# san-soucie/gdrf

Hardware: AMD Instinct MI355X
Metric: ELBO steps/sec (+ achieved HBM GB/s on K_nm) at N=1e6,M=512,K=10,V=50 (higher is better)
Workload: dtype f32; 1 GPU; configs[3] at 1 GPU(s): N=1000000 synthetic 2-D lattice (1000x1000), V=50, K=10, M=512 (32x16 grid inducing points), rbf kernel, Adam lr=1e-3, Trace_ELBO, 1 particle, jitter=1e-06, observations sharded over ranks; N=1000000, M=512, K=10, V=50, D=2, rows_per_rank=1000000, jitter_level=2, stores_T=False, mfma_mode=f16x3

## Files before the change

### gdrf_amd/csrc/gemm_tn_topics1.h

```cpp
#pragma once
#include <utility>
#include "gemm_tn_topics.h"

namespace gdrf {

template <int... Is, class F> __device__ __forceinline__ void static_for_impl(std::integer_sequence<int, Is...>, F&& f) {
  (f(std::integral_constant<int, Is>{}), ...);
}
template <int N, class F> __device__ __forceinline__ void static_for(F&& f) { static_for_impl(std::make_integer_sequence<int, N>{}, f); }

constexpr int TN1_CH = 64;
constexpr int TN1_XBLK = 1056;
constexpr int TN1_X_BYTES = 16 * TN1_XBLK;
constexpr int TN1_VROWS = 12;
constexpr int TN1_V_BYTES = TN1_VROWS * TN1_CH * 4;
constexpr int TN1_NBUF = 3;

__device__ __forceinline__ void glds4_asm(const void* gsrc, unsigned lds_dst) {
  asm volatile("s_mov_b32 m0, %1\n\ts_nop 0\n\tglobal_load_lds_dword %0, off" : : "v"(gsrc), "s"(lds_dst) : "memory");
}

__device__ __forceinline__ void glds4_asm_s(const void* sbase, unsigned voff, unsigned lds_dst) {
  asm volatile("s_mov_b32 m0, %2\n\ts_nop 0\n\tglobal_load_lds_dword %0, %1" : : "v"(voff), "s"(sbase), "s"(lds_dst) : "memory");
}

__global__ void tn1_scale_rows_kernel(const float* __restrict__ vbar, int64_t ldk, int64_t nrows, float* __restrict__ vs, int64_t lds,
                                      const float* __restrict__ sc, int sidx_v) {
  const int k = blockIdx.y;
  const float scale = sc[sidx_v + 2 * k];
  for (int64_t n = (int64_t)blockIdx.x * blockDim.x + threadIdx.x; n < lds; n += (int64_t)gridDim.x * blockDim.x)
    vs[(int64_t)k * lds + n] = n < nrows ? vbar[(int64_t)k * ldk + n] * scale : 0.0f;
}

constexpr int TN2_A_BYTES = 2 * 2 * 32 * 128 * 2;
constexpr int TN2_BUF = TN2_A_BYTES + TN1_X_BYTES + TN1_V_BYTES;
constexpr int TN2_DMA_PER_CHUNK = 15;
constexpr int tn2_lds_bytes() { return TN1_NBUF * TN2_BUF; }

__host__ __device__ inline int tn2_ntiles_half(int ncols) {
  const int nI = (ncols + 127) / 128, nJ = (ncols + 63) / 64;
  int t = 0;
  for (int I = 0; I < nI; ++I) t += (2 * I + 1 < nJ) ? 1 : 0;
  return t;
}
template <int AMIN>
__global__ __launch_bounds__(256, 1) void tn_topics_w2_kernel(TNTopicsArgs g) {
  using E = _Float16;
  using V8 = f16x8;
  using V4 = f16x4;
  constexpr int KT = TNT_KT, PIECE = 32 * 128, KA = 8;
  static_assert(KT == 10, "register plan below is for 10 topics");
  extern __shared__ __attribute__((aligned(16))) char smem[];
  const int tid = threadIdx.x, lane = tid & 63;
  const int w = __builtin_amdgcn_readfirstlane(tid >> 6);
  const int lr = lane & 15, lg = lane >> 4;
  const int kgroups = (g.K + KT - 1) / KT;
  const unsigned units = (unsigned)(g.ntiles * kgroups), bid = blockIdx.x;
  unsigned u; int sp;
  if ((g.nsplit & 7) == 0) { const unsigned idx = bid >> 3; sp = (int)(idx / units) * 8 + (int)(bid & 7u); u = idx % units; }
  else { sp = (int)(bid / units); u = bid % units; }
  const int tile = (int)(u % (unsigned)g.ntiles), gk = (int)(u / (unsigned)g.ntiles);
  int I = 0, J = tile;
  if (AMIN == 4) { I = tile; J = 2 * tile + 1; }
  else {
    const int nJ = (g.ncols + 63) / 64;
    for (;; ++I) { const int cnt = 2 * I + 1 < nJ ? 2 * I + 1 : nJ; if (J < cnt) break; J -= cnt; }
  }
  const int i0 = I * 128, j0 = J * 64;
  const int k0 = gk * KT, kg = min(KT, g.K - k0);
  const int64_t r0 = (int64_t)sp * g.rows_per_split;
  int64_t r1 = r0 + g.rows_per_split; if (r1 > g.nrows) r1 = g.nrows;
  const int nch = r0 < r1 ? (int)((r1 - r0 + TN1_CH - 1) / TN1_CH) : 0;
  const bool col_ok = (j0 + 16 * w) < g.ncols;
  const int bj = 2 * J + (w >> 1);

  f32x4 accA[KA][8], accV[KT - KA][8];
#pragma unroll
  for (int a = 0; a < 8; ++a) {
#pragma unroll
    for (int k = 0; k < KA; ++k) accA[k][a] = f32x4{0, 0, 0, 0};
#pragma unroll
    for (int k = 0; k < KT - KA; ++k) accV[k][a] = f32x4{0, 0, 0, 0};
  }

  const unsigned lds0 = lds_addr(smem);
  auto dma_edge = [&](int c, int buf) {
    const unsigned base = lds0 + (unsigned)(buf * TN2_BUF);
    const int64_t n0 = r0 + (int64_t)c * TN1_CH;
#pragma unroll
    for (int s = 0; s < 2; ++s)
#pragma unroll
      for (int h = 0; h < 2; ++h) {
        const int rb = w + 4 * h, k = 4 * rb + (lane >> 4);
        const int c8 = (lane & 15) ^ (tnb_code(k) << 1);
        int64_t n = n0 + 32 * s + k;
        n = n < g.nrows ? n : g.nrows - 1;
        const int col = (i0 + 8 * c8 < g.ncols) ? i0 + 8 * c8 : 0;
#pragma unroll
        for (int p = 0; p < 2; ++p)
          glds16_asm(g.Ah + p * g.a_stride + n * g.lda + col, base + (unsigned)((s * 2 + p) * PIECE * 2 + rb * 1024));
      }
    const int xcol = (j0 + 4 * (lane & 15) < g.ncols) ? j0 + 4 * (lane & 15) : 0;
#pragma unroll
    for (int t = 0; t < 4; ++t) {
      const int blk = 4 * w + t;
      int64_t n = n0 + 4 * blk + (lane >> 4);
      n = n < g.nrows ? n : g.nrows - 1;
      glds16_asm(g.B + n * g.ldb + xcol, base + (unsigned)(TN2_A_BYTES + blk * TN1_XBLK));
    }
#pragma unroll
    for (int t = 0; t < 3; ++t) {
      const int kk = w + 4 * t, ks = kk < kg ? kk : kg - 1;
      glds4_asm(g.vbar + (int64_t)(k0 + ks) * g.ldk + n0 + lane, base + (unsigned)(TN2_A_BYTES + TN1_X_BYTES + kk * TN1_CH * 4));
    }
  };
  unsigned voff_a, voff_x;
  {
    const int k = 4 * w + (lane >> 4);
    const int c8 = (lane & 15) ^ (tnb_code(k) << 1);
    const int col = (i0 + 8 * c8 < g.ncols) ? i0 + 8 * c8 : 0;
    voff_a = (unsigned)(((int64_t)(lane >> 4) * g.lda + col) * 2);
    const int xcol = (j0 + 4 * (lane & 15) < g.ncols) ? j0 + 4 * (lane & 15) : 0;
    voff_x = (unsigned)(((int64_t)(lane >> 4) * g.ldb + xcol) * 4);
  }
  const unsigned voff_v = (unsigned)lane * 4u;
  auto dma_is_edge = [&](int c) { return r0 + (int64_t)c * TN1_CH + TN1_CH > g.nrows; };
  auto dma_piece = [&](int c, int buf, int q) {
    const int64_t n0 = r0 + (int64_t)c * TN1_CH;
    const unsigned base = lds0 + (unsigned)(buf * TN2_BUF);
    if (q < 8) {
      const int s = q >> 2, h = (q >> 1) & 1, p = q & 1;
      glds16_asm_s(g.Ah + p * g.a_stride + (n0 + 32 * s + 16 * h + 4 * w) * g.lda, voff_a, base + (unsigned)((s * 2 + p) * PIECE * 2 + (w + 4 * h) * 1024));
    } else if (q < 12) {
      const int t = q - 8;
      glds16_asm_s(g.B + (n0 + 4 * (4 * w + t)) * g.ldb, voff_x, base + (unsigned)(TN2_A_BYTES + (4 * w + t) * TN1_XBLK));
    } else {
      const int kk = w + 4 * (q - 12), ks = kk < kg ? kk : kg - 1;
      glds4_asm_s(g.vbar + (int64_t)(k0 + ks) * g.ldk + n0, voff_v, base + (unsigned)(TN2_A_BYTES + TN1_X_BYTES + kk * TN1_CH * 4));
    }
  };
  auto dma = [&](int c, int buf) {
    if (dma_is_edge(c)) { dma_edge(c, buf); return; }
#pragma unroll
    for (int q = 0; q < TN2_DMA_PER_CHUNK; ++q) dma_piece(c, buf, q);
  };
  const int fq = lr >> 2, fp = lr & 3, fcode = ((lg & 1) << 2) | fq;
  const int fbase = (8 * lg + fq) * 32 + fp;
  auto frag = [&](const E* img, int g16) -> V8 {
    const int seg = fbase + ((g16 ^ fcode) << 2);
    const V4 lo = tr_read(img + seg * 4);
    const V4 hi = tr_read(img + (seg + 128) * 4);
    return __builtin_shufflevector(lo, hi, 0, 1, 2, 3, 4, 5, 6, 7);
  };
  const unsigned kmask = 0xffffe000u;
  const float k2048 = 2048.0f;
  auto split_piece = [&](int q, float xa, float xb, float va, float vb, float& y0, float& y1, float& h0, float& h1, unsigned& H, unsigned& L) {
    if (q == 0) asm volatile("v_mul_f32 %0, %2, %3\n\tv_mul_f32 %1, %4, %5" : "=&v"(y0), "=&v"(y1) : "v"(xa), "v"(va), "v"(xb), "v"(vb));
    if (q == 1) asm volatile("v_and_b32 %0, %2, %3\n\tv_and_b32 %1, %2, %4" : "=&v"(h0), "=&v"(h1) : "s"(kmask), "v"(y0), "v"(y1));
    if (q == 2) asm volatile("v_sub_f32 %0, %0, %2\n\tv_sub_f32 %1, %1, %3" : "+v"(y0), "+v"(y1) : "v"(h0), "v"(h1));
    if (q == 3) asm volatile("v_cvt_pkrtz_f16_f32 %0, %2, %3\n\tv_mul_f32 %1, %4, %1" : "=&v"(H), "+v"(y0) : "v"(h0), "v"(h1), "s"(k2048));
    if (q == 4) asm volatile("v_mul_f32 %1, %3, %1\n\tv_cvt_pk_f16_f32 %0, %2, %1" : "=&v"(L), "+v"(y1) : "v"(y0), "s"(k2048));
  };
  auto mfma_a = [&](f32x4& acc, const V8& a, const V8& b) { asm volatile("v_mfma_f32_16x16x32_f16 %0, %1, %2, %0" : "+a"(acc) : "v"(a), "v"(b)); };
  auto mfma_v = [&](f32x4& acc, const V8& a, const V8& b) { asm volatile("v_mfma_f32_16x16x32_f16 %0, %1, %2, %0" : "+v"(acc) : "v"(a), "v"(b)); };
  auto wait_next = [&](bool two_ahead) {
    if (two_ahead) asm volatile("s_waitcnt vmcnt(%0) lgkmcnt(0)" :: "n"(TN2_DMA_PER_CHUNK) : "memory");
    else asm volatile("s_waitcnt vmcnt(0) lgkmcnt(0)" ::: "memory");
  };

  if (nch > 0) {
    constexpr int NA = 8 - AMIN, NM = 3 * NA, NPS = NM - 2;
    dma(0, 0);
    if (nch > 1) dma(1, 1);
    wait_next(nch > 1);
    gdrf_raw_barrier();
    int buf = 0, bn = 2;
    for (int c = 0; c < nch; ++c) {
      const bool two = c + 2 < nch;
      const bool spread = two && !dma_is_edge(c + 2);
      if (two && !spread) dma_edge(c + 2, bn);
      const E* As = reinterpret_cast<const E*>(smem + buf * TN2_BUF);
      const float* xs = reinterpret_cast<const float*>(smem + buf * TN2_BUF + TN2_A_BYTES);
      const float* vt = reinterpret_cast<const float*>(smem + buf * TN2_BUF + TN2_A_BYTES + TN1_X_BYTES);
      V8 fah[8], fal[8], fa2[8];
#pragma unroll
      for (int a = AMIN; a < 8; ++a) { fah[a] = frag(As, a); fal[a] = frag(As + PIECE, a); }
      float xv[2][8];
#pragma unroll
      for (int s = 0; s < 2; ++s)
#pragma unroll
        for (int e = 0; e < 8; ++e) xv[s][e] = xs[(8 * s + 2 * lg + (e >> 2)) * (TN1_XBLK / 4) + (e & 3) * 64 + 16 * w + lr];
      constexpr int NST = 2 * KT;
      f32x4 vv[3][2];
      auto load_vv = [&](int t) {
        const int s = t / KT, k = t % KT;
        vv[t % 3][0] = *reinterpret_cast<const f32x4*>(vt + k * TN1_CH + 32 * s + 8 * lg);
        vv[t % 3][1] = *reinterpret_cast<const f32x4*>(vt + k * TN1_CH + 32 * s + 8 * lg + 4);
      };
      unsigned Hh[2][4], Ll[2][4];
      float y0, y1, h0, h1;
      auto piece = [&](int t, int q20) {
        const int s = t / KT, g2 = q20 / 5;
        const f32x4 v = vv[t % 3][g2 >> 1];
        split_piece(q20 % 5, xv[s][2 * g2], xv[s][2 * g2 + 1], v[2 * (g2 & 1)], v[2 * (g2 & 1) + 1], y0, y1, h0, h1, Hh[t & 1][g2], Ll[t & 1][g2]);
      };
      load_vv(0);
      load_vv(1);
#pragma unroll
      for (int a = AMIN; a < 8; ++a) fa2[a] = fah[a] * (E)0.00048828125f;
#pragma unroll
      for (int q = 0; q < 20; ++q) piece(0, q);
      typedef unsigned u32x4 __attribute__((ext_vector_type(4)));
      V8 fbh = __builtin_bit_cast(V8, u32x4{Hh[0][0], Hh[0][1], Hh[0][2], Hh[0][3]});
      V8 fbl = __builtin_bit_cast(V8, u32x4{Ll[0][0], Ll[0][1], Ll[0][2], Ll[0][3]});
      asm volatile("s_nop 1" : "+v"(fbh), "+v"(fbl));
      static_for<NST>([&](auto tc) {
        constexpr int t = decltype(tc)::value;
        constexpr int s = t / KT, k = t % KT;
        if (k == 0) {
          if (s == 1) {
#pragma unroll
            for (int a = AMIN; a < 8; ++a) { fah[a] = frag(As + 2 * PIECE, a); fal[a] = frag(As + 3 * PIECE, a); }
#pragma unroll
            for (int a = AMIN; a < 8; ++a) fa2[a] = fah[a] * (E)0.00048828125f;
          }
          if (AMIN == 0) asm volatile("s_nop 1" : "+v"(fa2[0]), "+v"(fa2[1]), "+v"(fa2[2]), "+v"(fa2[3]), "+v"(fa2[4]), "+v"(fa2[5]), "+v"(fa2[6]), "+v"(fa2[7]));
          else asm volatile("s_nop 1" : "+v"(fa2[4]), "+v"(fa2[5]), "+v"(fa2[6]), "+v"(fa2[7]));
        }
        if (t + 2 < NST) load_vv(t + 2);
        const V8 fbh_t = fbh, fbl_t = fbl;
        static_for<NM>([&](auto mc) {
          constexpr int m = decltype(mc)::value;
          constexpr int x = m / NA, a = AMIN + m % NA;
          const V8& fa = x == 0 ? fa2[a] : (x == 1 ? fal[a] : fah[a]);
          const V8& fb = x == 0 ? fbl_t : fbh_t;
          if (k < KA) mfma_a(accA[k < KA ? k : 0][a], fa, fb); else mfma_v(accV[k >= KA ? k - KA : 0][a], fa, fb);
          if (m < NPS && t + 1 < NST) {
#pragma unroll
            for (int q = m * 20 / NPS; q < (m + 1) * 20 / NPS; ++q) piece(t + 1, q);
          }
          if (m == NPS - 1 && t + 1 < NST) {
            fbh = __builtin_bit_cast(V8, u32x4{Hh[(t + 1) & 1][0], Hh[(t + 1) & 1][1], Hh[(t + 1) & 1][2], Hh[(t + 1) & 1][3]});
            fbl = __builtin_bit_cast(V8, u32x4{Ll[(t + 1) & 1][0], Ll[(t + 1) & 1][1], Ll[(t + 1) & 1][2], Ll[(t + 1) & 1][3]});
            asm volatile("" : "+v"(fbh), "+v"(fbl));
          }
          if (m == NM - 2 && spread && t < TN2_DMA_PER_CHUNK) dma_piece(c + 2, bn, t);
        });
      });
      wait_next(two);
      gdrf_raw_barrier();
      buf = buf == 2 ? 0 : buf + 1;
      bn = bn == 2 ? 0 : bn + 1;
    }
  }
  asm volatile("s_nop 15\n\ts_nop 15" ::: "memory");
  if (!col_ok) return;
  const float una = g.sc[g.sidx_a + 1];
#pragma unroll
  for (int k = 0; k < KT; ++k) {
    if (k < kg) {
      const float un = una * g.sc[g.sidx_v + 2 * (k0 + k) + 1];
      float* out = g.slab + ((int64_t)sp * g.K + k0 + k) * (int64_t)g.ncols * g.ncols;
#pragma unroll
      for (int a = 0; a < 8; ++a) {
        if (4 * I + (a >> 1) < bj) continue;
#pragma unroll
        for (int r = 0; r < 4; ++r) {
          const int i = i0 + 16 * a + 4 * lg + r;
          const int j = j0 + 16 * w + lr;
          const float v = k < KA ? accA[k < KA ? k : 0][a][r] : accV[k >= KA ? k - KA : 0][a][r];
          if (i < g.ncols && j < g.ncols) out[(int64_t)i * g.ncols + j] = v * un;
        }
      }
    }
  }
}

}
```

Measured before the change: 25.12 steps/s.

## Software-pipeline operand prefetch across chunk boundaries in topics GEMM

Hoists the fragment registers out of the chunk loop and prefetches the next chunk's A fragments, x values and v vectors from LDS during the current chunk's last MFMA steps. The wait and barrier move earlier, to step NST-2. This removes the per-chunk prologue where LDS reads and the split pieces ran with no MFMA overlap. In exchange, more registers stay live and the barrier placement is more delicate, with a risk of races or spills.

```diff
diff --git a/gdrf_amd/csrc/gemm_tn_topics1.h b/gdrf_amd/csrc/gemm_tn_topics1.h
--- a/gdrf_amd/csrc/gemm_tn_topics1.h
+++ b/gdrf_amd/csrc/gemm_tn_topics1.h
@@ -170,11 +170,50 @@
 
   if (nch > 0) {
     constexpr int NA = 8 - AMIN, NM = 3 * NA, NPS = NM - 2;
+    constexpr int NST = 2 * KT;
+    typedef unsigned u32x4 __attribute__((ext_vector_type(4)));
+    V8 fah[8], fal[8], fa2[8];
+    float xv[2][8];
+    f32x4 vv[3][2];
+    unsigned Hh[2][4], Ll[2][4];
+    float y0, y1, h0, h1;
+    V8 fbh, fbl;
+    auto xread = [&](const float* xs, int s, int e) {
+      return xs[(8 * s + 2 * lg + (e >> 2)) * (TN1_XBLK / 4) + (e & 3) * 64 + 16 * w + lr];
+    };
+    auto load_vv = [&](const float* vt, int t) {
+      const int s = t / KT, k = t % KT;
+      vv[t % 3][0] = *reinterpret_cast<const f32x4*>(vt + k * TN1_CH + 32 * s + 8 * lg);
+      vv[t % 3][1] = *reinterpret_cast<const f32x4*>(vt + k * TN1_CH + 32 * s + 8 * lg + 4);
+    };
+    auto piece = [&](int t, int q20) {
+      const int s = t / KT, g2 = q20 / 5;
+      const f32x4 v = vv[t % 3][g2 >> 1];
+      split_piece(q20 % 5, xv[s][2 * g2], xv[s][2 * g2 + 1], v[2 * (g2 & 1)], v[2 * (g2 & 1) + 1], y0, y1, h0, h1, Hh[t & 1][g2], Ll[t & 1][g2]);
+    };
     dma(0, 0);
     if (nch > 1) dma(1, 1);
     wait_next(nch > 1);
     gdrf_raw_barrier();
-    int buf = 0, bn = 2;
+    {
+      const E* As = reinterpret_cast<const E*>(smem);
+      const float* xs = reinterpret_cast<const float*>(smem + TN2_A_BYTES);
+      const float* vt = reinterpret_cast<const float*>(smem + TN2_A_BYTES + TN1_X_BYTES);
+#pragma unroll
+      for (int a = AMIN; a < 8; ++a) { fah[a] = frag(As, a); fal[a] = frag(As + PIECE, a); }
+#pragma unroll
+      for (int e = 0; e < 8; ++e) xv[0][e] = xread(xs, 0, e);
+      load_vv(vt, 0);
+      load_vv(vt, 1);
+#pragma unroll
+      for (int a = AMIN; a < 8; ++a) fa2[a] = fah[a] * (E)0.00048828125f;
+#pragma unroll
+      for (int q = 0; q < 20; ++q) piece(0, q);
+      fbh = __builtin_bit_cast(V8, u32x4{Hh[0][0], Hh[0][1], Hh[0][2], Hh[0][3]});
+      fbl = __builtin_bit_cast(V8, u32x4{Ll[0][0], Ll[0][1], Ll[0][2], Ll[0][3]});
+      asm volatile("s_nop 1" : "+v"(fbh), "+v"(fbl));
+    }
+    int buf = 0, b1 = 1, bn = 2;
     for (int c = 0; c < nch; ++c) {
       const bool two = c + 2 < nch;
       const bool spread = two && !dma_is_edge(c + 2);
@@ -182,75 +221,54 @@
       const E* As = reinterpret_cast<const E*>(smem + buf * TN2_BUF);
       const float* xs = reinterpret_cast<const float*>(smem + buf * TN2_BUF + TN2_A_BYTES);
       const float* vt = reinterpret_cast<const float*>(smem + buf * TN2_BUF + TN2_A_BYTES + TN1_X_BYTES);
-      V8 fah[8], fal[8], fa2[8];
-#pragma unroll
-      for (int a = AMIN; a < 8; ++a) { fah[a] = frag(As, a); fal[a] = frag(As + PIECE, a); }
-      float xv[2][8];
-#pragma unroll
-      for (int s = 0; s < 2; ++s)
-#pragma unroll
-        for (int e = 0; e < 8; ++e) xv[s][e] = xs[(8 * s + 2 * lg + (e >> 2)) * (TN1_XBLK / 4) + (e & 3) * 64 + 16 * w + lr];
-      constexpr int NST = 2 * KT;
-      f32x4 vv[3][2];
-      auto load_vv = [&](int t) {
-        const int s = t / KT, k = t % KT;
-        vv[t % 3][0] = *reinterpret_cast<const f32x4*>(vt + k * TN1_CH + 32 * s + 8 * lg);
-        vv[t % 3][1] = *reinterpret_cast<const f32x4*>(vt + k * TN1_CH + 32 * s + 8 * lg + 4);
-      };
-      unsigned Hh[2][4], Ll[2][4];
-      float y0, y1, h0, h1;
-      auto piece = [&](int t, int q20) {
-        const int s = t / KT, g2 = q20 / 5;
-        const f32x4 v = vv[t % 3][g2 >> 1];
-        split_piece(q20 % 5, xv[s][2 * g2], xv[s][2 * g2 + 1], v[2 * (g2 & 1)], v[2 * (g2 & 1) + 1], y0, y1, h0, h1, Hh[t & 1][g2], Ll[t & 1][g2]);
-      };
-      load_vv(0);
-      load_vv(1);
-#pragma unroll
-      for (int a = AMIN; a < 8; ++a) fa2[a] = fah[a] * (E)0.00048828125f;
-#pragma unroll
-      for (int q = 0; q < 20; ++q) piece(0, q);
-      typedef unsigned u32x4 __attribute__((ext_vector_type(4)));
-      V8 fbh = __builtin_bit_cast(V8, u32x4{Hh[0][0], Hh[0][1], Hh[0][2], Hh[0][3]});
-      V8 fbl = __builtin_bit_cast(V8, u32x4{Ll[0][0], Ll[0][1], Ll[0][2], Ll[0][3]});
-      asm volatile("s_nop 1" : "+v"(fbh), "+v"(fbl));
+      const E* As_n = reinterpret_cast<const E*>(smem + b1 * TN2_BUF);
+      const float* xs_n = reinterpret_cast<const float*>(smem + b1 * TN2_BUF + TN2_A_BYTES);
+      const float* vt_n = reinterpret_cast<const float*>(smem + b1 * TN2_BUF + TN2_A_BYTES + TN1_X_BYTES);
       static_for<NST>([&](auto tc) {
         constexpr int t = decltype(tc)::value;
         constexpr int s = t / KT, k = t % KT;
+        constexpr int tn = (t + 1) % NST;
         if (k == 0) {
-          if (s == 1) {
-#pragma unroll
-            for (int a = AMIN; a < 8; ++a) { fah[a] = frag(As + 2 * PIECE, a); fal[a] = frag(As + 3 * PIECE, a); }
-#pragma unroll
-            for (int a = AMIN; a < 8; ++a) fa2[a] = fah[a] * (E)0.00048828125f;
-          }
           if (AMIN == 0) asm volatile("s_nop 1" : "+v"(fa2[0]), "+v"(fa2[1]), "+v"(fa2[2]), "+v"(fa2[3]), "+v"(fa2[4]), "+v"(fa2[5]), "+v"(fa2[6]), "+v"(fa2[7]));
           else asm volatile("s_nop 1" : "+v"(fa2[4]), "+v"(fa2[5]), "+v"(fa2[6]), "+v"(fa2[7]));
         }
-        if (t + 2 < NST) load_vv(t + 2);
+        if (t == NST - 2) {
+          wait_next(two);
+          gdrf_raw_barrier();
+        }
+        if (t < 8) xv[1][t] = xread(xs, 1, t);
+        if (t + 2 < NST) load_vv(vt, t + 2); else load_vv(vt_n, t + 2 - NST);
         const V8 fbh_t = fbh, fbl_t = fbl;
+        const E* Ah_nx = s == 0 ? As + 2 * PIECE : As_n;
         static_for<NM>([&](auto mc) {
           constexpr int m = decltype(mc)::value;
           constexpr int x = m / NA, a = AMIN + m % NA;
           const V8& fa = x == 0 ? fa2[a] : (x == 1 ? fal[a] : fah[a]);
           const V8& fb = x == 0 ? fbl_t : fbh_t;
           if (k < KA) mfma_a(accA[k < KA ? k : 0][a], fa, fb); else mfma_v(accV[k >= KA ? k - KA : 0][a], fa, fb);
-          if (m < NPS && t + 1 < NST) {
-#pragma unroll
-            for (int q = m * 20 / NPS; q < (m + 1) * 20 / NPS; ++q) piece(t + 1, q);
+          if (m < NPS) {
+#pragma unroll
+            for (int q = m * 20 / NPS; q < (m + 1) * 20 / NPS; ++q) piece(tn, q);
           }
-          if (m == NPS - 1 && t + 1 < NST) {
-            fbh = __builtin_bit_cast(V8, u32x4{Hh[(t + 1) & 1][0], Hh[(t + 1) & 1][1], Hh[(t + 1) & 1][2], Hh[(t + 1) & 1][3]});
-            fbl = __builtin_bit_cast(V8, u32x4{Ll[(t + 1) & 1][0], Ll[(t + 1) & 1][1], Ll[(t + 1) & 1][2], Ll[(t + 1) & 1][3]});
+          if (k == KT - 1) {
+            if (x == 0) fa2[a] = frag(Ah_nx, a);
+            if (x == 1) {
+              fal[a] = frag(Ah_nx + PIECE, a);
+              fa2[a] = fa2[a] * (E)0.00048828125f;
+              asm volatile("" : "+v"(fa2[a]));
+            }
+            if (x == 2) fah[a] = frag(Ah_nx, a);
+          }
+          if (t == NST - 2 && m < 8) xv[0][m] = xread(xs_n, 0, m);
+          if (m == NPS - 1) {
+            fbh = __builtin_bit_cast(V8, u32x4{Hh[tn & 1][0], Hh[tn & 1][1], Hh[tn & 1][2], Hh[tn & 1][3]});
+            fbl = __builtin_bit_cast(V8, u32x4{Ll[tn & 1][0], Ll[tn & 1][1], Ll[tn & 1][2], Ll[tn & 1][3]});
             asm volatile("" : "+v"(fbh), "+v"(fbl));
           }
           if (m == NM - 2 && spread && t < TN2_DMA_PER_CHUNK) dma_piece(c + 2, bn, t);
         });
       });
-      wait_next(two);
-      gdrf_raw_barrier();
-      buf = buf == 2 ? 0 : buf + 1;
-      bn = bn == 2 ? 0 : bn + 1;
+      buf = b1; b1 = bn; bn = bn == 2 ? 0 : bn + 1;
     }
   }
   asm volatile("s_nop 15\n\ts_nop 15" ::: "memory");
```

Result: no change. 25.08 steps/s (-0.1%).
